# pgvector/pgvector

Measured on AMD Instinct MI355X. Metric: QPS @ recall@10 (IVFFlat, 1M x 1536d), higher is better.
Workload: dtype f32

## Files before the change

### pgvector_amd/csrc/kernels_query.hip

```cpp
#include "pgv_device.h"
#include "pgv_select.h"

#include <type_traits>

namespace pgv {

namespace {

constexpr int kQThreads = kSelThreads;
constexpr int kQWaves = kQThreads / kWave;
constexpr int kMaxBatchLists = 256;
constexpr int kHeadCap = 1024;

template <typename T, int METRIC, int NCH> struct WholeRows {
    Raw16 q[NCH];
    __device__ __forceinline__ void load_query(const char *qp, int lane) {
#pragma unroll
        for (int c = 0; c < NCH; c++) q[c] = load16(qp + ((size_t)c * kWave + lane) * sizeof(Raw16));
    }
    __device__ __forceinline__ float pair(const char *a, const char *b, int lane) const {
        Raw16 ra[NCH], rb[NCH];
#pragma unroll
        for (int c = 0; c < NCH; c++) ra[c] = load16(a + ((size_t)c * kWave + lane) * sizeof(Raw16));
#pragma unroll
// ... 290 lines not shown
        } else {
            out_dist[o] = INFINITY;
            if (out_slot) out_slot[o] = -1;
            if (out_tid) out_tid[o] = ~0ull;
        }
    }
    if (stats && threadIdx.x == 0) {
        atomicAdd(&stats[0], (double)m);
        atomicAdd(&stats[1], (double)m);
        atomicAdd(&stats[5], (double)m);
    }
}

constexpr int kRecheckCap = 256;

template <typename T, bool DOT = false>
__global__ __launch_bounds__(kQThreads) void batch_recheck_kernel(
    const char *__restrict__ vectors, const uint64_t *__restrict__ tids, int nvec, int lg,
    const char *__restrict__ queries, int kprime, int k, const float *__restrict__ approx_val,
    const int64_t *__restrict__ cand_pos, const int64_t *__restrict__ cand_slot,
    const int64_t *__restrict__ list_off, const int32_t *__restrict__ probe_lists,
    const int64_t *__restrict__ probe_off, int probes,
    const int64_t *__restrict__ seg_start, int64_t fixed_len,
    const unsigned *__restrict__ row_norm_max, ScanBound bound, const float *__restrict__ eps_add, int nq,
    float *__restrict__ out_dist, int64_t *__restrict__ out_slot, uint64_t *__restrict__ out_tid,
    int32_t *__restrict__ out_i32, int32_t *__restrict__ flags, float *__restrict__ pair_t, PlanEmit emit) {
    static_assert(!DOT || std::is_same<T, float>::value, "pair terms: fp32 rows");
    __shared__ float exact[kRecheckCap];
    __shared__ float dots[DOT ? kRecheckCap : 1];
    __shared__ __attribute__((aligned(16))) unsigned long long ent[kRecheckCap];
    const int q = blockIdx.x;
    const size_t row_bytes = (size_t)nvec * sizeof(Raw16);
    const int64_t m = seg_start ? seg_start[q + 1] - seg_start[q] : fixed_len;
    const int ncand = (int)(m < kprime ? m : (int64_t)kprime);
    const int kk = ncand < k ? ncand : k;
    const float *av = approx_val + (size_t)q * kprime;
    __shared__ float qn_part[kQWaves];
    {
        const char *qrow = queries + (size_t)q * row_bytes;
        float a = 0.f;
        for (int v = threadIdx.x; v < nvec; v += kQThreads) {
            const Raw16 x = load16(qrow + (size_t)v * sizeof(Raw16));
            a = accum_slice<T, 1>(a, x, x);
        }
        for (int m2 = 32; m2 > 0; m2 >>= 1) a += __shfl_xor(a, m2);
        if ((threadIdx.x & (kWave - 1)) == 0) qn_part[threadIdx.x >> 6] = a;
    }
    __syncthreads();
    float qn = 0.f;
    for (int w = 0; w < kQWaves; w++) qn += qn_part[w];
    const float rn = __uint_as_float(*row_norm_max);
    const float cross = 2.f * sqrtf(qn * rn);
    const float eps = 1.001f * (bound.g_sq * (qn + rn + cross) + bound.g_dot * cross + bound.g_norm * rn +
                                (eps_add ? eps_add[q] : 0.f));
    unsigned band = 0u;
    if (kk > 0) {
        const float edge = av[kk - 1] + 2.f * eps;
        band = float_to_key(edge + bound.g_ref * fabsf(edge + qn));
    }
    const int cnt = __syncthreads_count((int)threadIdx.x < ncand && float_to_key(av[threadIdx.x]) <= band);
    __shared__ int64_t slots[kRecheckCap];
    if ((int)threadIdx.x < cnt) {
        const int64_t p = cand_pos[(size_t)q * kprime + threadIdx.x];
        int64_t slot = p;
        if (cand_slot) {
            slot = cand_slot[(size_t)q * kprime + threadIdx.x];
        } else {
            const int64_t *off = probe_off + (size_t)q * probes;
            int lo = 0, hi = probes - 1;
            while (lo < hi) {
                const int mid = (lo + hi + 1) >> 1;
                if (off[mid] <= p)
                    lo = mid;
                else
                    hi = mid - 1;
            }
            slot = list_off[probe_lists[(size_t)q * probes + lo]] + (p - off[lo]);
        }
        slots[threadIdx.x] = slot;
    }
    __syncthreads();
    if constexpr (DOT)
        score_rows_dot([&](int64_t j) { return vectors + (size_t)slots[j] * row_bytes; }, 0, cnt,
                       queries + (size_t)q * row_bytes, nvec, lg, exact, dots);
    else
        score_rows<T, 0, 0>([&](int64_t j) { return vectors + (size_t)slots[j] * row_bytes; }, 0, cnt,
                            queries + (size_t)q * row_bytes, nvec, lg, exact);
    __syncthreads();
    if ((int)threadIdx.x < kRecheckCap)
        ent[threadIdx.x] = (int)threadIdx.x < cnt
                               ? ((unsigned long long)float_to_key(exact[threadIdx.x]) << 32) |
                                     (unsigned)cand_pos[(size_t)q * kprime + threadIdx.x]
                               : ~0ull;
    __syncthreads();
    const unsigned long long mine = ent[threadIdx.x];
    const int64_t my_slot = (int)threadIdx.x < cnt ? slots[threadIdx.x] : -1;
    int rank = 0;
    {
        const ulonglong2 *e2 = reinterpret_cast<const ulonglong2 *>(ent);
        const int n2 = (cnt + 1) / 2;
#pragma unroll 8
        for (int j = 0; j < n2; j++) {
            const ulonglong2 o = e2[j];
            rank += o.x < mine ? 1 : 0;
            rank += o.y < mine ? 1 : 0;
        }
    }
// ... 392 lines not shown
    float *cand_val = nullptr;
    int64_t *cand_pos = nullptr;
    int32_t *flags = nullptr;
    int carve(DBuf &buf, int nq, int kprime) {
        const size_t nk = (size_t)nq * kprime;
        const size_t a1 = (sizeof(float) * nk + 15) & ~(size_t)15, a2 = a1 + sizeof(int64_t) * nk;
        PGV_TRY(buf.ensure(a2 + sizeof(int32_t) * (2 * (size_t)nq + 1)));
        cand_val = buf.as<float>();
        cand_pos = reinterpret_cast<int64_t *>(buf.as<char>() + a1);
        flags = reinterpret_cast<int32_t *>(buf.as<char>() + a2);
        return PGV_OK;
    }
};
}

int launch_exact_tail(pgv_ctx *ctx, const ExactTail &t, DBuf &scratch) {
    if (t.nq <= 0) return PGV_OK;
    const ExactRows &xr = t.rows;
    const bool dense = t.dense();
    if (dense ? (t.fixed_len <= 0 || t.probe_off || t.seg_start || t.probes != 0)
              : (t.fixed_len != 0 || !t.probe_off || !t.seg_start || t.probes < 1))
        PGV_FAIL(PGV_ERR_ARG, "exact tail: a list plan or one dense run");
    if (t.kprime > kRecheckCap || t.k > t.kprime)
        PGV_FAIL(PGV_ERR_ARG, "exact tail: k' = %d outside k..%d", t.kprime, kRecheckCap);
    if (t.pair_t && xr.dtype != PGV_F32) PGV_FAIL(PGV_ERR_ARG, "exact tail: pair terms are for fp32 rows");
    static_assert(kWide >= kRecheckCap, "k <= k' <= kWide: batch_fix_kernel's emit");
    if (t.emit.cnt && !(dense && t.pair_t && t.out_i32 && t.emit.probe_off && t.emit.seg_len && t.emit.list_off))
        PGV_FAIL(PGV_ERR_ARG, "exact tail: the plan is counted where the pair terms are written");
    ApproxScratch sc;
    PGV_TRY(sc.carve(scratch, t.nq, t.kprime));
    const int64_t *cand_slot = dense ? sc.cand_pos : nullptr;
    const int64_t *seg_start = dense ? nullptr : t.seg_start;
    const int64_t fixed_len = dense ? t.fixed_len : 0;
    PGV_TRY(launch_topk_segments(ctx, t.approx, seg_start, t.nq, fixed_len, t.kprime, sc.cand_val, sc.cand_pos,
                                 sc.flags + t.nq, t.emit.cnt, t.emit.cnt ? 2 * (int)fixed_len : 0));
#define PGV_RECHECK(T, DOT)                                                                                          \
    hipLaunchKernelGGL((batch_recheck_kernel<T, DOT>), dim3(t.nq), dim3(kQThreads), 0, ctx->stream,                   \
                       static_cast<const char *>(xr.vectors), xr.tids, xr.geom.nvec, xr.geom.lpr_log2,                \
                       static_cast<const char *>(t.queries), t.kprime, t.k, sc.cand_val, sc.cand_pos, cand_slot,      \
                       xr.list_offsets, t.probe_lists, t.probe_off, t.probes, seg_start, fixed_len, xr.norm_max,      \
                       t.bound, t.eps_add, t.nq, t.out_dist, t.out_slot, t.out_tid, t.out_i32, sc.flags, t.pair_t,    \
                       t.emit)
    if (t.pair_t)
        PGV_RECHECK(float, true);
    else if (xr.dtype == PGV_F32)
        PGV_RECHECK(float, false);
    else
        PGV_RECHECK(__half, false);
#undef PGV_RECHECK
    PGV_HIP(hipGetLastError());
    double *stats = (ctx->profiling && ctx->stats_dev.p) ? ctx->stats_dev.as<double>() : nullptr;
    int kp = 2;
    while (kp < t.k) kp <<= 1;
    const int cap = kp > kFastCap ? kp : kFastCap;
    const size_t lds = (size_t)cap * 8 + sizeof(SelShared);
    const int grid = t.nq < ctx->num_cus ? t.nq : ctx->num_cus;
#define PGV_FIX(T)                                                                                                    \
    hipLaunchKernelGGL(batch_fix_kernel<T>, dim3(grid), dim3(kQThreads), lds, ctx->stream,                            \
                       static_cast<const char *>(xr.vectors), xr.list_offsets, xr.tids, xr.geom.nvec,                 \
                       xr.geom.lpr_log2, static_cast<const char *>(t.queries), t.probe_lists, t.probe_off, t.probes,  \
                       seg_start, fixed_len, sc.flags, t.nq, t.approx, t.k, kp, cap, xr.norm_max, t.bound, t.eps_add, \
                       ctx->no_widen ? 0 : 1, t.out_dist, t.out_slot, t.out_tid, t.out_i32, stats, t.pair_t, t.emit)
    if (xr.dtype == PGV_F32)
// ... 10 lines not shown
```

### pgvector_amd/csrc/kernels_select.hip

```cpp
#include "pgv_device.h"
#include "pgv_select.h"

namespace pgv {

namespace {


__global__ void plan_count_kernel(const int32_t *__restrict__ probe_lists,
                                  const int64_t *__restrict__ list_off, int nq, int probes,
                                  int *__restrict__ cnt, int64_t *__restrict__ probe_off,
                                  int64_t *__restrict__ seg_len) {
    const int q = blockIdx.x * blockDim.x + threadIdx.x;
    if (q >= nq) return;
    int64_t run = 0;
    for (int p = 0; p < probes; p++) {
        const int l = probe_lists[(size_t)q * probes + p];
        probe_off[(size_t)q * probes + p] = run;
        run += list_off[l + 1] - list_off[l];
        atomicAdd(&cnt[l], 1);
    }
    seg_len[q] = run;
}

template <typename F>
// ... 127 lines not shown
        ScanTask task;
        task.row0 = list_off[l] + (int64_t)c * rows_per_task;
        const int64_t left = len - (int64_t)c * rows_per_task;
        task.nrows = (int)(left < rows_per_task ? left : rows_per_task);
        task.pair0 = (int)(pair_start[l] + (int64_t)g * qt);
        const int pl = cnt[l] - g * qt;
        task.npairs = pl < qt ? pl : qt;
        task.pad = ng > 1 ? 1 : 0;
        tasks[t] = task;
    }
}

__global__ void plan_tasks_kernel(const int *__restrict__ cnt, const int64_t *__restrict__ list_off,
                                  const int64_t *__restrict__ pair_start,
                                  const int64_t *__restrict__ task_start, int nlists, int qt,
                                  int rows_per_task, ScanTask *__restrict__ tasks) {
    plan_tasks_body((int64_t)blockIdx.x * blockDim.x + threadIdx.x, (int64_t)gridDim.x * blockDim.x, cnt, list_off,
                    pair_start, task_start, nlists, qt, rows_per_task, tasks);
}

__global__ void plan_pairs_tasks_kernel(const int32_t *__restrict__ probe_lists, const int64_t *__restrict__ list_off,
                                        const int64_t *__restrict__ probe_off, const int64_t *__restrict__ seg_start,
                                        const int64_t *__restrict__ pair_start, const int64_t *__restrict__ task_start,
                                        const int *__restrict__ cnt, int *__restrict__ fill, int nq, int probes, int nlists,
                                        int qt, int rows_per_task, const float *__restrict__ pair_t, int pair_blocks,
                                        ScanPair *__restrict__ pairs, ScanTask *__restrict__ tasks) {
    if ((int)blockIdx.x < pair_blocks)
        plan_pairs_body((int64_t)blockIdx.x * blockDim.x + threadIdx.x, probe_lists, list_off, probe_off, seg_start,
                        pair_start, fill, nq, probes, pair_t, pairs);
    else
        plan_tasks_body((int64_t)(blockIdx.x - pair_blocks) * blockDim.x + threadIdx.x,
                        (int64_t)(gridDim.x - pair_blocks) * blockDim.x, cnt, list_off, pair_start, task_start, nlists, qt,
                        rows_per_task, tasks);
}

__device__ __forceinline__ bool dist_before(float a, float b) { return float_to_key(a) < float_to_key(b); }


__global__ __launch_bounds__(kSelThreads) void topk_kernel(
    const float *__restrict__ vals, const int64_t *__restrict__ seg_start, int64_t fixed_len,
    int k, int kp, int cap, float *__restrict__ out_val, int64_t *__restrict__ out_pos,
// ... 141 lines not shown
    const size_t nb = npairs + (size_t)nq + (size_t)nq + 1 + 2 * ((size_t)nlists + 1) + 3;
    PGV_TRY(ctx->plan_b.ensure(sizeof(int64_t) * nb));
    pb->cnt = ctx->plan_a.as<int>();
    pb->fill = pb->cnt + nlists;
    pb->probe_off = ctx->plan_b.as<int64_t>();
    pb->seg_len = pb->probe_off + npairs;
    pb->seg_start = pb->seg_len + nq;
    pb->pair_start = pb->seg_start + nq + 1;
    pb->task_start = pb->pair_start + nlists + 1;
    pb->totals = pb->task_start + nlists + 1;
    return PGV_OK;
}

int launch_plan_batch(pgv_ctx *ctx, const pgv_index *ix, const int32_t *probe_lists, int nq,
                      int probes, int qt, int rows_per_task, bool read_totals, PlanResult *res, const float *pair_t,
                      bool counted) {
    const int nlists = ix->nlists;
    const size_t npairs = (size_t)nq * probes;

    int64_t max_chunks = 0, sum_chunks = 0;
    for (int l = 0; l < nlists; l++) {
        const int64_t nc = (ix->h_offsets[l + 1] - ix->h_offsets[l] + rows_per_task - 1) / rows_per_task;
        sum_chunks += nc;
        if (nc > max_chunks) max_chunks = nc;
    }
    res->ntasks_bound = max_chunks * (int64_t)(npairs / qt) + sum_chunks;
    res->out_bound = (int64_t)nq * ix->len_prefix[probes];
    if (res->ntasks_bound > 0x7fffffff) PGV_FAIL(PGV_ERR_ARG, "plan: too many tasks");

    PlanBuffers pb;
    PGV_TRY(plan_batch_reserve(ctx, nlists, nq, probes, &pb));
// ... 8 lines not shown
    const unsigned task_blocks = (unsigned)(want < 1 ? 1 : (want > cap ? cap : want));
    const unsigned pair_blocks = (unsigned)((npairs + 255) / 256);
    res->ntasks = res->ntasks_bound;
    res->total_out = res->out_bound;

    if (counted) {
        double *acc = nullptr;
        if (read_totals) {
            PGV_TRY(ctx->stats_dev.ensure(8 * sizeof(double)));
            acc = ctx->stats_dev.as<double>();
        }
        hipLaunchKernelGGL(plan_scan_kernel, dim3(1), dim3(1024), 0, ctx->stream, cnt, ix->list_offsets, seg_len, nq, nlists,
                           qt, rows_per_task, seg_start, pair_start, task_start, totals, acc);
        hipLaunchKernelGGL(plan_pairs_tasks_kernel, dim3(pair_blocks + task_blocks), dim3(256), 0, ctx->stream, probe_lists,
                           ix->list_offsets, probe_off, seg_start, pair_start, task_start, cnt, fill, nq, probes, nlists, qt,
                           rows_per_task, pair_t, (int)pair_blocks, ctx->pairs.as<ScanPair>(), tasks);
        PGV_HIP(hipGetLastError());
    } else {
        PGV_HIP(hipMemsetAsync(cnt, 0, sizeof(int) * 2 * (size_t)nlists, ctx->stream));
        hipLaunchKernelGGL(plan_count_kernel, dim3((nq + 255) / 256), dim3(256), 0, ctx->stream,
                           probe_lists, ix->list_offsets, nq, probes, cnt, probe_off, seg_len);
        hipLaunchKernelGGL(plan_scan_kernel, dim3(1), dim3(1024), 0, ctx->stream, cnt,
                           ix->list_offsets, seg_len, nq, nlists, qt, rows_per_task, seg_start,
                           pair_start, task_start, totals, static_cast<double *>(nullptr));
        hipLaunchKernelGGL(plan_pairs_kernel, dim3(pair_blocks), dim3(256), 0,
                           ctx->stream, probe_lists, ix->list_offsets, probe_off, seg_start,
                           pair_start, fill, nq, probes, pair_t, ctx->pairs.as<ScanPair>());
        hipLaunchKernelGGL(plan_tasks_kernel, dim3(task_blocks), dim3(256), 0,
                           ctx->stream, cnt, ix->list_offsets, pair_start, task_start, nlists, qt, rows_per_task, tasks);
        PGV_HIP(hipGetLastError());
        if (read_totals) {
            PGV_TRY(ctx->stats_dev.ensure(8 * sizeof(double)));
            hipLaunchKernelGGL(plan_stats_kernel, dim3(1), dim3(256), 0, ctx->stream, cnt,
                               ix->list_offsets, totals, nlists, qt, ctx->stats_dev.as<double>());
            PGV_HIP(hipGetLastError());
        }
    }
    res->tasks = tasks;
    res->pairs = ctx->pairs.as<ScanPair>();
    res->ntasks_dev = reinterpret_cast<int *>(totals + 2);
    res->seg_start = seg_start;
    res->probe_off = probe_off;
    res->pair_start = pair_start;
    return PGV_OK;
// ... 41 lines not shown
```

### pgvector_amd/csrc/kernels_shadow.hip

```cpp
#include "pgv_device.h"

#include <cfloat>

namespace pgv {

namespace {

__device__ __forceinline__ int list_of_row(const int64_t *__restrict__ list_off, int nlists, int64_t r) {
    int lo = 0, hi = nlists - 1;
    while (lo < hi) {
        const int mid = (lo + hi + 1) >> 1;
        if (list_off[mid] <= r)
            lo = mid;
        else
            hi = mid - 1;
    }
    return lo;
}

__device__ __forceinline__ int scale_for(float m) {
    if (!(m > 0.f) || !isfinite(m)) return 0;
    int e;
    (void)frexpf(m, &e);
    return e - 14;
// ... 105 lines not shown
            qq[e & 3] = fma(xi, xi, qq[e & 3]);
            dd[e & 3] = fma(xi - back, xi - back, dd[e & 3]);
            hh[e & 3] = fma(back, back, hh[e & 3]);
        }
        out.v[e] = v;
    }
    *reinterpret_cast<uint4 *>(h + 8 * c) = out.w;
}

__global__ __launch_bounds__(256) void shadow_query_kernel(const float *__restrict__ queries, int nq, int ld, int ld16,
                                                           ShadowTerms st, RankShadowTerms rt,
                                                           const float *__restrict__ center_norm_max,
                                                           const float *__restrict__ row_norm_max,
                                                           __half *__restrict__ qcast, float *__restrict__ qscale,
                                                           float *__restrict__ qeps, float *__restrict__ cscale,
                                                           float *__restrict__ ceps) {
    const int q = (int)(blockIdx.x * 4 + (threadIdx.x >> 6));
    if (q >= nq) return;
    const int lane = threadIdx.x & (kWave - 1);
    const float *x = queries + (size_t)q * ld;
    __half *h = qcast + (size_t)q * ld16;
    const int nchunks = ld16 / 8;
    const bool in_regs = nchunks <= kWave * kCastChunks;
    CastChunk reg[kCastChunks];
    float m = 0.f;
    if (in_regs) {
#pragma unroll
        for (int j = 0; j < kCastChunks; j++) {
            const int c = lane + j * kWave;
            reg[j] = cast_chunk_load(x, c < nchunks ? c : nchunks, ld);
        }
// ... 92 lines not shown
    hipLaunchKernelGGL(shadow_build_kernel, grid, dim3(256), 0, ctx->stream, static_cast<const float *>(rows),
                       static_cast<const float *>(centers), list_off, nlists, n, g32.ld, g16.ld, max_bits, static_cast<__half *>(shadow), ep);
    PGV_HIP(hipGetLastError());
    return PGV_OK;
}

int shadow_scale_of(float max_abs) {
    if (!(max_abs > 0.f) || !std::isfinite(max_abs)) return 0;
    int e;
    (void)std::frexp(max_abs, &e);
    return e - 14;
}

int launch_shadow_query(pgv_ctx *ctx, const RowGeom &g32, const RowGeom &g16, const void *queries, int nq,
                        const ShadowTerms &st, const RankShadowTerms &rt, const float *center_norm_max,
                        const float *row_norm_max, void *qcast, float *qscale, float *qeps, float *cscale, float *ceps) {
    if (nq <= 0) return PGV_OK;
    hipLaunchKernelGGL(shadow_query_kernel, dim3((unsigned)((nq + 3) / 4)), dim3(256), 0, ctx->stream,
                       static_cast<const float *>(queries), nq, g32.ld, g16.ld, st, rt, center_norm_max, row_norm_max,
                       static_cast<__half *>(qcast), qscale, qeps, cscale, ceps);
    PGV_HIP(hipGetLastError());
    return PGV_OK;
}

int launch_shadow_pairs(pgv_ctx *ctx, const RowGeom &g32, const void *queries, const void *centers,
                        const int64_t *pair_start, int nlists, int64_t npairs, ScanPair *pairs) {
    if (npairs <= 0) return PGV_OK;
    hipLaunchKernelGGL(shadow_pair_kernel, dim3((unsigned)((npairs + 3) / 4)), dim3(256), 0, ctx->stream,
                       static_cast<const float *>(queries), static_cast<const float *>(centers), pair_start, nlists, npairs,
                       g32.ld, pairs);
    PGV_HIP(hipGetLastError());
    return PGV_OK;
}

}
// ... 1 lines not shown
```

### pgvector_amd/csrc/pgv_abi_ivf.hip

```cpp
#include "pgv_abi_common.h"

extern "C" {


namespace {
struct IndexLayout {
    size_t centers, vectors, offsets, tids, row_norms, center_norms, bytes;
    bool has_tids, has_norms;
};
IndexLayout index_layout(int nlists, int64_t n, size_t row_bytes, bool has_tids, bool l2) {
    auto up = [](size_t v) { return (v + 255) & ~(size_t)255; };
    IndexLayout L{};
    size_t at = 0;
    L.centers = at; at = up(at + (size_t)nlists * row_bytes);
    L.vectors = at; at = up(at + (size_t)(n > 0 ? n : 1) * row_bytes);
    L.offsets = at; at = up(at + sizeof(int64_t) * ((size_t)nlists + 1));
    L.has_tids = has_tids;
    L.tids = at; if (has_tids) at = up(at + sizeof(uint64_t) * (size_t)n);
    L.has_norms = l2;
    L.row_norms = at; if (l2 && n > 0) at = up(at + sizeof(float) * ((size_t)n + 1));
    L.center_norms = at; if (l2) at = up(at + sizeof(float) * ((size_t)nlists + 1));
    L.bytes = at;
    return L;
}
// ... 92 lines not shown
        ix->cshadow_P = Pc * (1.0 + 1e-9);
    }
    return PGV_OK;
}

struct ShadowBatch {
    void *qcast = nullptr;
    float *qscale = nullptr, *qeps = nullptr;
    float *cscale = nullptr, *ceps = nullptr;
    float *pair_t = nullptr;
    bool scan_follows = false;
    bool cast_for_scan = false;
    bool pairs_done = false;
};

int shadow_batch_cast(pgv_index *ix, const void *q_dev, int nq, int probes, bool for_rank, bool for_scan, ShadowBatch *sb) {
    pgv_ctx *ctx = ix->ctx;
    const RowGeom &g16 = ix->shadow_geom;
    const size_t qb = ((size_t)nq * g16.ld * sizeof(uint16_t) + 255) & ~(size_t)255;
    PGV_TRY(ctx->sh_q.ensure(qb + sizeof(float) * (size_t)nq * (4 + (size_t)probes)));
    sb->qcast = ctx->sh_q.p;
    sb->qscale = reinterpret_cast<float *>(ctx->sh_q.as<char>() + qb);
    sb->qeps = sb->qscale + nq;
    sb->cscale = sb->qeps + nq;
    sb->ceps = sb->cscale + nq;
    sb->pair_t = sb->ceps + nq;
    constexpr double u = 5.9604644775390625e-8;
    ShadowTerms st{};
    st.s = ix->shadow_s;
    st.E = ix->shadow_E;
    st.P = ix->shadow_P;
    st.g_dot = gamma_n(shadow_chain_length(g16) + 4.0, u);
    st.g_pair = gamma_n((double)pair_chain_length(ix->geom), u);
    st.g_cn = shadow_band(ix->geom.ld, 0.f, u).g_norm;
    RankShadowTerms rt{};
    rt.s = ix->cshadow_s;
    rt.E = ix->cshadow_E;
    rt.P = ix->cshadow_P;
    rt.g_dot = st.g_dot;
    rt.g_cn = st.g_cn;
    PGV_TRY(launch_shadow_query(ctx, ix->geom, g16, q_dev, nq, st, rt, ix->center_norms + ix->nlists,
                                ix->row_norms + ix->nrows, sb->qcast, for_scan ? sb->qscale : nullptr,
                                for_scan ? sb->qeps : nullptr, for_rank ? sb->cscale : nullptr,
                                for_rank ? sb->ceps : nullptr));
    sb->cast_for_scan = for_scan;
    return PGV_OK;
}

template <typename Fill>
int index_create(pgv_ctx *ctx, pgv_metric metric, pgv_dtype dtype, int dim, int nlists, const std::vector<int64_t> &off,
                 bool has_tids, Fill fill, pgv_index **out) {
    const int64_t n = off[nlists];
    pgv_index *ix = new (std::nothrow) pgv_index();
    if (!ix) PGV_FAIL(PGV_ERR_NOMEM, "out of host memory");
    ix->ctx = ctx;
    ix->refs = new (std::nothrow) int(1);
    if (!ix->refs) {
        delete ix;
        PGV_FAIL(PGV_ERR_NOMEM, "out of host memory");
// ... 599 lines not shown
        const int64_t cd_stride = ((int64_t)ix->nlists + 7) / 4 * 4;
        PGV_TRY(ctx->dist_mat.ensure(sizeof(float) * (size_t)nq * cd_stride));
        return launch_multi_rank(ctx, ix, q_dev, nq, ctx->dist_mat.as<float>(), cd_stride, maxprobes, out_lists_dev,
                                 out_dist_dev);
    }
    int cand = maxprobes + 16 < ix->nlists ? maxprobes + 16 : ix->nlists;
    const int rank_env = rank_shadow_env();
    const bool rank_sh = ix->metric == PGV_L2SQ && ix->cshadow && ix->dtype == PGV_F32 && rank_env != 0 && shadow_env() != 0;
    if (rank_sh && maxprobes + 54 <= 256) cand = maxprobes + 54 < ix->nlists ? maxprobes + 54 : ix->nlists;
    const bool mfma = nq >= 128 && ix->nlists >= 64 && !ctx->no_mfma_scan &&
                      (ix->metric == PGV_NEG_IP || (ix->metric == PGV_L2SQ && ix->center_norms && cand <= 256));
    if (mfma && ix->metric == PGV_L2SQ) {
        ShadowBatch own;
        if (!sb) sb = &own;
        const bool scan_follows = sb->scan_follows;
        if (rank_sh) {
            PGV_TRY(shadow_batch_cast(ix, q_dev, nq, maxprobes, true, scan_follows, sb));
            PGV_TRY(dense_scan(ctx, ix->metric, PGV_F16, ix->shadow_geom, ix->cshadow, ix->nlists, sb->qcast, nq, ix->nlists,
                               mat, true, ix->center_norms, nullptr, sb->cscale));
        } else {
            PGV_TRY(dense_scan(ctx, ix->metric, ix->dtype, ix->geom, ix->centers, ix->nlists, q_dev, nq, ix->nlists, mat,
                               true, ix->center_norms, nullptr));
        }
        ExactTail tail;
        tail.pair_t = (rank_sh && rank_env == 1 && scan_follows) ? sb->pair_t : nullptr;
        PlanBuffers pbuf;
        if (tail.pair_t) {
            PGV_TRY(plan_batch_reserve(ctx, ix->nlists, nq, maxprobes, &pbuf));
            tail.emit = {pbuf.cnt, pbuf.probe_off, pbuf.seg_len, ix->list_offsets};
        }
        tail.rows = {ix->centers, nullptr, nullptr, ix->geom, ix->dtype,
                     reinterpret_cast<const unsigned *>(ix->center_norms + ix->nlists)};
        tail.queries = q_dev;
        tail.nq = nq;
        tail.kprime = cand;
        tail.k = maxprobes;
        tail.approx = mat;
        tail.fixed_len = ix->nlists;
        tail.bound = scan_bound_chain(ctx, ix->geom.ld, scan_chain_length(ix->geom, ix->dtype, false));
        if (rank_sh) tail.bound = shadow_band(ix->geom.ld, tail.bound.g_ref);
        tail.eps_add = rank_sh ? sb->ceps : nullptr;
        tail.out_dist = dist;
        tail.out_i32 = out_lists_dev;
        PGV_TRY(launch_exact_tail(ctx, tail, ctx->ms_b));
// ... 184 lines not shown
        PGV_TRY(launch_multi_scan(ctx, ix, q_dev, nq, probe_lists, probes, bound, ctx->plan_d.as<float>(), seg_stride, k,
                                  od.as<float>(), os.as<int64_t>(), ot.as<uint64_t>()));
        PGV_TRY(timer.end());
        PGV_TRY(scan_turn_end(ctx));
        bool need = false;
        PGV_TRY(od.finish(ctx, &need));
        PGV_TRY(os.finish(ctx, &need));
        PGV_TRY(ot.finish(ctx, &need));
        return sync_if(ctx, need);
    }
    ShadowBatch own;
    if (!sb) sb = &own;
    if (path.shadow && !sb->cast_for_scan) PGV_TRY(shadow_batch_cast(ix, q_dev, nq, probes, false, true, sb));
    const float *pair_t = (path.shadow && sb->pairs_done) ? sb->pair_t : nullptr;
    PlanResult plan;
    PGV_TRY(launch_plan_batch(ctx, ix, probe_lists, nq, probes, path.qt, path.rows_per_task, ctx->profiling, &plan, pair_t,
                              pair_t != nullptr));
    if (path.shadow) {
        if (!pair_t)
            PGV_TRY(launch_shadow_pairs(ctx, ix->geom, q_dev, ix->centers, plan.pair_start, ix->nlists, (int64_t)nq * probes,
                                        plan.pairs));
        ctx->scan_shadow_queries += nq;
    }

    PGV_TRY(ctx->plan_d.ensure(sizeof(float) * (size_t)(plan.out_bound > 0 ? plan.out_bound : 1)));
    float *seg_vals = ctx->plan_d.as<float>();
    if (plan.ntasks_bound > 0) {
        PGV_TRY(scan_turn_begin(ctx));
        ScanTimer timer{ctx};
        PGV_TRY(timer.begin(0.0, 0.0));
        if (path.shadow)
            PGV_TRY(launch_mfma_scan(ctx, ix->metric, PGV_F16, ix->shadow_geom, ix->shadow, sb->qcast, plan.tasks,
// ... 26 lines not shown
        tail.queries = q_dev;
        tail.nq = nq;
        tail.kprime = approx_candidates(k);
        tail.k = k;
        tail.approx = seg_vals;
        tail.probe_lists = probe_lists;
        tail.probe_off = plan.probe_off;
        tail.probes = probes;
        tail.seg_start = plan.seg_start;
        tail.bound = scan_bound_chain(ctx, ix->geom.ld, scan_chain_length(ix->geom, ix->dtype, path.wide));
        if (path.shadow) tail.bound = shadow_band(ix->geom.ld, tail.bound.g_ref);
        tail.eps_add = path.shadow ? sb->qeps : nullptr;
        tail.out_dist = od.as<float>();
        tail.out_slot = os.as<int64_t>();
        tail.out_tid = ot.as<uint64_t>();
        PGV_TRY(launch_exact_tail(ctx, tail, ctx->ms_a));
    } else {
        PGV_TRY(launch_topk_segments(ctx, seg_vals, plan.seg_start, nq, 0, k, od.as<float>(), pos));
        PGV_TRY(launch_positions_to_slots(ctx, ix, probe_lists, plan.probe_off, nq, probes, k, pos,
                                          os.as<int64_t>(), ot.as<uint64_t>()));
    }
    bool need = false;
    PGV_TRY(od.finish(ctx, &need));
    PGV_TRY(os.finish(ctx, &need));
    PGV_TRY(ot.finish(ctx, &need));
    return sync_if(ctx, need);
}

int scan_batch_dev(pgv_index *ix, const void *q_dev, int nq, const int32_t *probe_lists, int probes, int k, float *out_dist,
                   int64_t *out_slot, uint64_t *out_tid) {
// ... 284 lines not shown
```

### pgvector_amd/csrc/pgv_internal.h

```cpp
#pragma once

#include <hip/hip_runtime.h>

#include <cstdint>
#include <cstdio>
#include <cstdlib>
#include <cstring>
#include <cmath>
#include <vector>

#include "../../include/pgv_hip.h"

namespace pgv {

void set_error(const char *fmt, ...) __attribute__((format(printf, 1, 2)));

#define PGV_FAIL(code, ...)            \
    do {                               \
        ::pgv::set_error(__VA_ARGS__); \
        return (code);                 \
    } while (0)

#define PGV_HIP(call)                                                                  \
    do {                                                                               \
// ... 352 lines not shown
int mfma_scan_queries_per_task();
int launch_mfma_dense(pgv_ctx *ctx, pgv_metric metric, pgv_dtype dtype, const RowGeom &g, const void *rows, int64_t n,
                      const void *queries, int nq, const float *row_norms, float *out, int64_t out_stride);
int dense_chain_length(const RowGeom &g, pgv_dtype dtype);
int launch_row_norms(pgv_ctx *ctx, pgv_dtype dtype, const RowGeom &g, const void *rows, int64_t n, float *out,
                     unsigned *max_bits);
int launch_mfma_scan(pgv_ctx *ctx, pgv_metric metric, pgv_dtype dtype, const RowGeom &g, const void *rows,
                     const void *queries, const ScanTask *tasks, const int *ntasks_dev, int ntasks_bound,
                     const ScanPair *pairs, const float *row_norms, const float *query_norms, float *out, bool stream_rows,
                     int queries_per_task = 32, const float *shadow_scale = nullptr);
int launch_shadow_build(pgv_ctx *ctx, const RowGeom &g32, const RowGeom &g16, const void *rows, const void *centers,
                        const int64_t *list_off, int nlists, int64_t n, void *shadow, void *words);
int shadow_scale_of(float max_abs);
int shadow_chain_length(const RowGeom &g16);
int scan_chain_length(const RowGeom &g, pgv_dtype dtype, bool wide);
int launch_shadow_query(pgv_ctx *ctx, const RowGeom &g32, const RowGeom &g16, const void *queries, int nq,
                        const ShadowTerms &st, const RankShadowTerms &rt, const float *center_norm_max,
                        const float *row_norm_max, void *qcast, float *qscale, float *qeps, float *cscale, float *ceps);
int launch_shadow_pairs(pgv_ctx *ctx, const RowGeom &g32, const void *queries, const void *centers,
                        const int64_t *pair_start, int nlists, int64_t npairs, ScanPair *pairs);
int mfma_scan_queries_per_task_wide();

int launch_gather_words(pgv_ctx *ctx, const void *src, int words_per_row, int64_t nrows, const int64_t *idx, int n,
                        uint32_t *out);
size_t build_sort_scratch_bytes(int64_t n, int key_bits);
int launch_build_order(pgv_ctx *ctx, const int32_t *lists, int64_t n, int nlists, unsigned long long *keys_tmp,
                       unsigned long long *keys_sorted, unsigned long long *counts, int64_t *offsets, int *bad,
                       void *sort_scratch, size_t sort_scratch_bytes);
int launch_build_gather(pgv_ctx *ctx, const void *src_rows, const unsigned long long *keys_sorted, int64_t n, int nvec,
                        void *dst_rows, const uint64_t *src_tids, uint64_t *dst_tids);

struct PlanResult {
    ScanTask *tasks = nullptr;
// ... 8 lines not shown
    int64_t *pair_start = nullptr;
};
struct PlanBuffers {
    int *cnt = nullptr, *fill = nullptr;
    int64_t *probe_off = nullptr, *seg_len = nullptr;
    int64_t *seg_start = nullptr, *pair_start = nullptr, *task_start = nullptr, *totals = nullptr;
};
int plan_batch_reserve(pgv_ctx *ctx, int nlists, int nq, int probes, PlanBuffers *pb);
struct PlanEmit {
    int *cnt = nullptr;
    int64_t *probe_off = nullptr, *seg_len = nullptr;
    const int64_t *list_off = nullptr;
};
int launch_plan_batch(pgv_ctx *ctx, const pgv_index *ix, const int32_t *probe_lists, int nq,
                      int probes, int qt, int rows_per_task, bool read_totals, PlanResult *res,
                      const float *pair_t = nullptr, bool counted = false);
int launch_topk_segments(pgv_ctx *ctx, const float *vals, const int64_t *seg_start, int nseg,
                         int64_t fixed_len, int k, float *out_val, int64_t *out_pos, int32_t *zero_word = nullptr,
                         int32_t *zero_range = nullptr, int zero_n = 0);
int launch_positions_to_slots(pgv_ctx *ctx, const pgv_index *ix, const int32_t *probe_lists,
                              const int64_t *probe_off, int nq, int probes, int k,
                              const int64_t *pos, int64_t *out_slot, uint64_t *out_tid);
struct ExactRows {
    const void *vectors;
    const uint64_t *tids;
    const int64_t *list_offsets;
    pgv::RowGeom geom;
    pgv_dtype dtype;
    const unsigned *norm_max;
};
struct ExactTail {
// ... 4 lines not shown
    int k = 0;
    float *approx = nullptr;
    const int32_t *probe_lists = nullptr;
    const int64_t *probe_off = nullptr;
    int probes = 0;
    const int64_t *seg_start = nullptr;
    int64_t fixed_len = 0;
    ScanBound bound{};
    const float *eps_add = nullptr;
    float *out_dist = nullptr;
    int64_t *out_slot = nullptr;
    uint64_t *out_tid = nullptr;
    int32_t *out_i32 = nullptr;
    float *pair_t = nullptr;
    PlanEmit emit;
    bool dense() const { return probe_lists == nullptr; }
};
int launch_exact_tail(pgv_ctx *ctx, const ExactTail &t, DBuf &scratch);
int launch_iota_slots(pgv_ctx *ctx, const pgv_index *ix, const int32_t *lists_dev, int nlists,
                      const int64_t *probe_off, int64_t *out_slot);

int query_max_batch_lists();
int query_head_cap();
size_t query_head_bytes(int head);
int launch_query_stage(pgv_ctx *ctx, const void *src_pinned, void *dst_dev, int nvec);
int launch_multi_rank(pgv_ctx *ctx, const pgv_index *ix, const void *q_dev, int nq, float *cdist, int64_t cd_stride,
                      int max_probes, int32_t *out_lists, float *out_dist);
int launch_multi_scan(pgv_ctx *ctx, const pgv_index *ix, const void *q_dev, int nq, const int32_t *probe_lists, int nprobes,
                      int64_t rows_bound, float *seg, int64_t seg_stride, int k, float *out_dist, int64_t *out_slot,
                      uint64_t *out_tid);
int launch_query_iota(pgv_ctx *ctx, int32_t *out, int n);
int launch_one_query_rows(pgv_ctx *ctx, pgv_metric metric, pgv_dtype dtype, const RowGeom &g, const void *rows, int n,
// ... 44 lines not shown
```

Baseline: 1.373 million.

## Fuse segment top-k selection into the exact recheck kernel

Folds the per-query segment top-k selection into the batch recheck kernel, so candidates come straight from shared memory instead of a separate launch writing cand_val/cand_pos to global scratch. The zeroing of the flag and count words moves into earlier kernels (shadow query cast, plan tasks). Probe offsets and list bases are staged in LDS for the binary search, and query-norm loads are hoisted ahead of the selection. This removes a kernel launch and a global round trip per batch, at the cost of more dynamic shared memory per workgroup and a more complex kernel with possibly lower occupancy.

```diff
diff --git a/pgvector_amd/csrc/kernels_query.hip b/pgvector_amd/csrc/kernels_query.hip
--- a/pgvector_amd/csrc/kernels_query.hip
+++ b/pgvector_amd/csrc/kernels_query.hip
@@ -328,7 +328,10 @@
 
 constexpr int kRecheckCap = 256;
 
-template <typename T, bool DOT = false>
+constexpr int kProbeLds = 128;
+constexpr int kQnHoist = 2;
+
+template <typename T, bool DOT = false, bool FUSED = false>
 __global__ __launch_bounds__(kQThreads) void batch_recheck_kernel(
     const char *__restrict__ vectors, const uint64_t *__restrict__ tids, int nvec, int lg,
     const char *__restrict__ queries, int kprime, int k, const float *__restrict__ approx_val,
@@ -338,22 +341,67 @@
     const int64_t *__restrict__ seg_start, int64_t fixed_len,
     const unsigned *__restrict__ row_norm_max, ScanBound bound, const float *__restrict__ eps_add, int nq,
     float *__restrict__ out_dist, int64_t *__restrict__ out_slot, uint64_t *__restrict__ out_tid,
-    int32_t *__restrict__ out_i32, int32_t *__restrict__ flags, float *__restrict__ pair_t, PlanEmit emit) {
+    int32_t *__restrict__ out_i32, int32_t *__restrict__ flags, float *__restrict__ pair_t, PlanEmit emit, int kp, int cap) {
     static_assert(!DOT || std::is_same<T, float>::value, "pair terms: fp32 rows");
+    static_assert(kQThreads == kSelThreads && kRecheckCap <= kQThreads, "one workgroup selects and rechecks a query");
+    extern __shared__ __attribute__((aligned(16))) char smem[];
     __shared__ float exact[kRecheckCap];
     __shared__ float dots[DOT ? kRecheckCap : 1];
     __shared__ __attribute__((aligned(16))) unsigned long long ent[kRecheckCap];
+    __shared__ int64_t poff[FUSED ? kProbeLds : 1], pbase[FUSED ? kProbeLds : 1];
     const int q = blockIdx.x;
     const size_t row_bytes = (size_t)nvec * sizeof(Raw16);
-    const int64_t m = seg_start ? seg_start[q + 1] - seg_start[q] : fixed_len;
+    const int64_t seg_base = seg_start ? seg_start[q] : (int64_t)q * fixed_len;
+    const int64_t m = seg_start ? seg_start[q + 1] - seg_base : fixed_len;
     const int ncand = (int)(m < kprime ? m : (int64_t)kprime);
     const int kk = ncand < k ? ncand : k;
     const float *av = approx_val + (size_t)q * kprime;
+    const bool dense = FUSED ? probe_lists == nullptr : cand_slot != nullptr;
+    const bool lds_probes = FUSED && !dense && probes <= kProbeLds;
+    float av_mine = INFINITY, av_edge = INFINITY;
+    int64_t pos_mine = -1;
     __shared__ float qn_part[kQWaves];
     {
         const char *qrow = queries + (size_t)q * row_bytes;
         float a = 0.f;
-        for (int v = threadIdx.x; v < nvec; v += kQThreads) {
+        int v = threadIdx.x;
+        if constexpr (FUSED) {
+            Raw16 x[kQnHoist];
+#pragma unroll
+            for (int h = 0; h < kQnHoist; h++) {
+                const int at = v + h * kQThreads;
+                x[h] = load16(qrow + (size_t)(at < nvec ? at : 0) * sizeof(Raw16));
+            }
+            int64_t off_r = 0;
+            int32_t list_r = 0;
+            if (lds_probes && (int)threadIdx.x < probes) {
+                off_r = probe_off[(size_t)q * probes + threadIdx.x];
+                list_r = probe_lists[(size_t)q * probes + threadIdx.x];
+            }
+            unsigned long long *sel_ent = reinterpret_cast<unsigned long long *>(smem);
+            SelShared *sel = reinterpret_cast<SelShared *>(smem + (size_t)cap * 8);
+            block_topk_auto(approx_val + seg_base, m, kprime, kp, cap, sel_ent, sel);
+            __syncthreads();
+            if (lds_probes && (int)threadIdx.x < probes) {
+                poff[threadIdx.x] = off_r;
+                pbase[threadIdx.x] = list_off[list_r];
+            }
+            auto value_of = [&](int i) {
+                const unsigned long long e = sel_ent[i];
+                return (e != ~0ull && i < ncand) ? key_to_float((unsigned)(e >> 32)) : INFINITY;
+            };
+            if ((int)threadIdx.x < kprime) {
+                const unsigned long long e = sel_ent[threadIdx.x];
+                av_mine = value_of((int)threadIdx.x);
+                pos_mine = (e != ~0ull && (int)threadIdx.x < ncand) ? (int64_t)(unsigned)(e & 0xffffffffu) : -1;
+            }
+            if (kk > 0) av_edge = value_of(kk - 1);
+#pragma unroll
+            for (int h = 0; h < kQnHoist; h++)
+                if (v + h * kQThreads < nvec) a = accum_slice<T, 1>(a, x[h], x[h]);
+            v += kQnHoist * kQThreads;
+        }
+        for (; v < nvec; v += kQThreads) {
             const Raw16 x = load16(qrow + (size_t)v * sizeof(Raw16));
             a = accum_slice<T, 1>(a, x, x);
         }
@@ -369,16 +417,29 @@
                                 (eps_add ? eps_add[q] : 0.f));
     unsigned band = 0u;
     if (kk > 0) {
-        const float edge = av[kk - 1] + 2.f * eps;
+        const float edge = (FUSED ? av_edge : av[kk - 1]) + 2.f * eps;
         band = float_to_key(edge + bound.g_ref * fabsf(edge + qn));
     }
-    const int cnt = __syncthreads_count((int)threadIdx.x < ncand && float_to_key(av[threadIdx.x]) <= band);
+    if constexpr (!FUSED)
+        if ((int)threadIdx.x < ncand) av_mine = av[threadIdx.x];
+    const int cnt = __syncthreads_count((int)threadIdx.x < ncand && float_to_key(av_mine) <= band);
     __shared__ int64_t slots[kRecheckCap];
     if ((int)threadIdx.x < cnt) {
-        const int64_t p = cand_pos[(size_t)q * kprime + threadIdx.x];
+        if constexpr (!FUSED) pos_mine = cand_pos[(size_t)q * kprime + threadIdx.x];
+        const int64_t p = pos_mine;
         int64_t slot = p;
-        if (cand_slot) {
-            slot = cand_slot[(size_t)q * kprime + threadIdx.x];
+        if (dense) {
+            if constexpr (!FUSED) slot = cand_slot[(size_t)q * kprime + threadIdx.x];
+        } else if (lds_probes) {
+            int lo = 0, hi = probes - 1;
+            while (lo < hi) {
+                const int mid = (lo + hi + 1) >> 1;
+                if (poff[mid] <= p)
+                    lo = mid;
+                else
+                    hi = mid - 1;
+            }
+            slot = pbase[lo] + (p - poff[lo]);
         } else {
             const int64_t *off = probe_off + (size_t)q * probes;
             int lo = 0, hi = probes - 1;
@@ -403,8 +464,7 @@
     __syncthreads();
     if ((int)threadIdx.x < kRecheckCap)
         ent[threadIdx.x] = (int)threadIdx.x < cnt
-                               ? ((unsigned long long)float_to_key(exact[threadIdx.x]) << 32) |
-                                     (unsigned)cand_pos[(size_t)q * kprime + threadIdx.x]
+                               ? ((unsigned long long)float_to_key(exact[threadIdx.x]) << 32) | (unsigned)pos_mine
                                : ~0ull;
     __syncthreads();
     const unsigned long long mine = ent[threadIdx.x];
@@ -827,6 +887,21 @@
 };
 }
 
+bool exact_tail_fused() {
+    static const bool on = [] {
+        const char *e = getenv("PGV_TAIL_FUSED");
+        return e ? atoi(e) != 0 : true;
+    }();
+    return on;
+}
+
+int exact_tail_reserve(DBuf &scratch, int nq, int32_t **count) {
+    ApproxScratch sc;
+    PGV_TRY(sc.carve(scratch, nq, 0));
+    *count = sc.flags + nq;
+    return PGV_OK;
+}
+
 int launch_exact_tail(pgv_ctx *ctx, const ExactTail &t, DBuf &scratch) {
     if (t.nq <= 0) return PGV_OK;
     const ExactRows &xr = t.rows;
@@ -840,26 +915,41 @@
     static_assert(kWide >= kRecheckCap, "k <= k' <= kWide: batch_fix_kernel's emit");
     if (t.emit.cnt && !(dense && t.pair_t && t.out_i32 && t.emit.probe_off && t.emit.seg_len && t.emit.list_off))
         PGV_FAIL(PGV_ERR_ARG, "exact tail: the plan is counted where the pair terms are written");
+    const bool fused = exact_tail_fused() && t.cleared_count != nullptr;
     ApproxScratch sc;
-    PGV_TRY(sc.carve(scratch, t.nq, t.kprime));
-    const int64_t *cand_slot = dense ? sc.cand_pos : nullptr;
+    PGV_TRY(sc.carve(scratch, t.nq, fused ? 0 : t.kprime));
+    if (fused && t.cleared_count != sc.flags + t.nq)
+        PGV_FAIL(PGV_ERR_STATE, "exact tail: the scratch moved after its flagged-query count was cleared");
     const int64_t *seg_start = dense ? nullptr : t.seg_start;
     const int64_t fixed_len = dense ? t.fixed_len : 0;
-    PGV_TRY(launch_topk_segments(ctx, t.approx, seg_start, t.nq, fixed_len, t.kprime, sc.cand_val, sc.cand_pos,
-                                 sc.flags + t.nq, t.emit.cnt, t.emit.cnt ? 2 * (int)fixed_len : 0));
-#define PGV_RECHECK(T, DOT)                                                                                          \
-    hipLaunchKernelGGL((batch_recheck_kernel<T, DOT>), dim3(t.nq), dim3(kQThreads), 0, ctx->stream,                   \
+    int skp = 2;
+    while (skp < t.kprime) skp <<= 1;
+    const int scap = skp > kFastCap ? skp : kFastCap;
+    const size_t slds = fused ? (size_t)scap * 8 + sizeof(SelShared) : 0;
+    const int64_t *cand_slot = (dense && !fused) ? sc.cand_pos : nullptr;
+    if (!fused)
+        PGV_TRY(launch_topk_segments(ctx, t.approx, seg_start, t.nq, fixed_len, t.kprime, sc.cand_val, sc.cand_pos,
+                                     sc.flags + t.nq, t.emit.cnt, t.emit.cnt ? 2 * (int)fixed_len : 0));
+#define PGV_RECHECK(T, DOT, FUSED)                                                                                   \
+    hipLaunchKernelGGL((batch_recheck_kernel<T, DOT, FUSED>), dim3(t.nq), dim3(kQThreads), slds, ctx->stream,         \
                        static_cast<const char *>(xr.vectors), xr.tids, xr.geom.nvec, xr.geom.lpr_log2,                \
-                       static_cast<const char *>(t.queries), t.kprime, t.k, sc.cand_val, sc.cand_pos, cand_slot,      \
-                       xr.list_offsets, t.probe_lists, t.probe_off, t.probes, seg_start, fixed_len, xr.norm_max,      \
-                       t.bound, t.eps_add, t.nq, t.out_dist, t.out_slot, t.out_tid, t.out_i32, sc.flags, t.pair_t,    \
-                       t.emit)
-    if (t.pair_t)
-        PGV_RECHECK(float, true);
-    else if (xr.dtype == PGV_F32)
-        PGV_RECHECK(float, false);
-    else
-        PGV_RECHECK(__half, false);
+                       static_cast<const char *>(t.queries), t.kprime, t.k, FUSED ? t.approx : sc.cand_val,           \
+                       sc.cand_pos, cand_slot, xr.list_offsets, t.probe_lists, t.probe_off, t.probes, seg_start,      \
+                       fixed_len, xr.norm_max, t.bound, t.eps_add, t.nq, t.out_dist, t.out_slot, t.out_tid,           \
+                       t.out_i32, sc.flags, t.pair_t, t.emit, skp, scap)
+#define PGV_RECHECK_T(FUSED)              \
+    if (t.pair_t)                         \
+        PGV_RECHECK(float, true, FUSED);  \
+    else if (xr.dtype == PGV_F32)         \
+        PGV_RECHECK(float, false, FUSED); \
+    else                                  \
+        PGV_RECHECK(__half, false, FUSED)
+    if (fused) {
+        PGV_RECHECK_T(true);
+    } else {
+        PGV_RECHECK_T(false);
+    }
+#undef PGV_RECHECK_T
 #undef PGV_RECHECK
     PGV_HIP(hipGetLastError());
     double *stats = (ctx->profiling && ctx->stats_dev.p) ? ctx->stats_dev.as<double>() : nullptr;
diff --git a/pgvector_amd/csrc/kernels_select.hip b/pgvector_amd/csrc/kernels_select.hip
--- a/pgvector_amd/csrc/kernels_select.hip
+++ b/pgvector_amd/csrc/kernels_select.hip
@@ -165,7 +165,8 @@
 __global__ void plan_tasks_kernel(const int *__restrict__ cnt, const int64_t *__restrict__ list_off,
                                   const int64_t *__restrict__ pair_start,
                                   const int64_t *__restrict__ task_start, int nlists, int qt,
-                                  int rows_per_task, ScanTask *__restrict__ tasks) {
+                                  int rows_per_task, ScanTask *__restrict__ tasks, int32_t *__restrict__ zero_word) {
+    if (zero_word && blockIdx.x == 0 && threadIdx.x == 0) *zero_word = 0;
     plan_tasks_body((int64_t)blockIdx.x * blockDim.x + threadIdx.x, (int64_t)gridDim.x * blockDim.x, cnt, list_off,
                     pair_start, task_start, nlists, qt, rows_per_task, tasks);
 }
@@ -175,7 +176,9 @@
                                         const int64_t *__restrict__ pair_start, const int64_t *__restrict__ task_start,
                                         const int *__restrict__ cnt, int *__restrict__ fill, int nq, int probes, int nlists,
                                         int qt, int rows_per_task, const float *__restrict__ pair_t, int pair_blocks,
-                                        ScanPair *__restrict__ pairs, ScanTask *__restrict__ tasks) {
+                                        ScanPair *__restrict__ pairs, ScanTask *__restrict__ tasks,
+                                        int32_t *__restrict__ zero_word) {
+    if (zero_word && blockIdx.x == 0 && threadIdx.x == 0) *zero_word = 0;
     if ((int)blockIdx.x < pair_blocks)
         plan_pairs_body((int64_t)blockIdx.x * blockDim.x + threadIdx.x, probe_lists, list_off, probe_off, seg_start,
                         pair_start, fill, nq, probes, pair_t, pairs);
@@ -347,7 +350,7 @@
 
 int launch_plan_batch(pgv_ctx *ctx, const pgv_index *ix, const int32_t *probe_lists, int nq,
                       int probes, int qt, int rows_per_task, bool read_totals, PlanResult *res, const float *pair_t,
-                      bool counted) {
+                      bool counted, int32_t *zero_word) {
     const int nlists = ix->nlists;
     const size_t npairs = (size_t)nq * probes;
 
@@ -386,7 +389,7 @@
                            qt, rows_per_task, seg_start, pair_start, task_start, totals, acc);
         hipLaunchKernelGGL(plan_pairs_tasks_kernel, dim3(pair_blocks + task_blocks), dim3(256), 0, ctx->stream, probe_lists,
                            ix->list_offsets, probe_off, seg_start, pair_start, task_start, cnt, fill, nq, probes, nlists, qt,
-                           rows_per_task, pair_t, (int)pair_blocks, ctx->pairs.as<ScanPair>(), tasks);
+                           rows_per_task, pair_t, (int)pair_blocks, ctx->pairs.as<ScanPair>(), tasks, zero_word);
         PGV_HIP(hipGetLastError());
     } else {
         PGV_HIP(hipMemsetAsync(cnt, 0, sizeof(int) * 2 * (size_t)nlists, ctx->stream));
@@ -399,7 +402,8 @@
                            ctx->stream, probe_lists, ix->list_offsets, probe_off, seg_start,
                            pair_start, fill, nq, probes, pair_t, ctx->pairs.as<ScanPair>());
         hipLaunchKernelGGL(plan_tasks_kernel, dim3(task_blocks), dim3(256), 0,
-                           ctx->stream, cnt, ix->list_offsets, pair_start, task_start, nlists, qt, rows_per_task, tasks);
+                           ctx->stream, cnt, ix->list_offsets, pair_start, task_start, nlists, qt, rows_per_task, tasks,
+                           zero_word);
         PGV_HIP(hipGetLastError());
         if (read_totals) {
             PGV_TRY(ctx->stats_dev.ensure(8 * sizeof(double)));
diff --git a/pgvector_amd/csrc/kernels_shadow.hip b/pgvector_amd/csrc/kernels_shadow.hip
--- a/pgvector_amd/csrc/kernels_shadow.hip
+++ b/pgvector_amd/csrc/kernels_shadow.hip
@@ -143,7 +143,10 @@
                                                            const float *__restrict__ row_norm_max,
                                                            __half *__restrict__ qcast, float *__restrict__ qscale,
                                                            float *__restrict__ qeps, float *__restrict__ cscale,
-                                                           float *__restrict__ ceps) {
+                                                           float *__restrict__ ceps, StreamClear clear) {
+    if (clear.word && blockIdx.x == 0 && threadIdx.x == 0) *clear.word = 0;
+    if (clear.range)
+        for (int i = (int)(blockIdx.x * 256 + threadIdx.x); i < clear.n; i += (int)(gridDim.x * 256)) clear.range[i] = 0;
     const int q = (int)(blockIdx.x * 4 + (threadIdx.x >> 6));
     if (q >= nq) return;
     const int lane = threadIdx.x & (kWave - 1);
@@ -266,11 +269,12 @@
 
 int launch_shadow_query(pgv_ctx *ctx, const RowGeom &g32, const RowGeom &g16, const void *queries, int nq,
                         const ShadowTerms &st, const RankShadowTerms &rt, const float *center_norm_max,
-                        const float *row_norm_max, void *qcast, float *qscale, float *qeps, float *cscale, float *ceps) {
+                        const float *row_norm_max, void *qcast, float *qscale, float *qeps, float *cscale, float *ceps,
+                        StreamClear clear) {
     if (nq <= 0) return PGV_OK;
     hipLaunchKernelGGL(shadow_query_kernel, dim3((unsigned)((nq + 3) / 4)), dim3(256), 0, ctx->stream,
                        static_cast<const float *>(queries), nq, g32.ld, g16.ld, st, rt, center_norm_max, row_norm_max,
-                       static_cast<__half *>(qcast), qscale, qeps, cscale, ceps);
+                       static_cast<__half *>(qcast), qscale, qeps, cscale, ceps, clear);
     PGV_HIP(hipGetLastError());
     return PGV_OK;
 }
diff --git a/pgvector_amd/csrc/pgv_abi_ivf.hip b/pgvector_amd/csrc/pgv_abi_ivf.hip
--- a/pgvector_amd/csrc/pgv_abi_ivf.hip
+++ b/pgvector_amd/csrc/pgv_abi_ivf.hip
@@ -130,7 +130,8 @@
     bool pairs_done = false;
 };
 
-int shadow_batch_cast(pgv_index *ix, const void *q_dev, int nq, int probes, bool for_rank, bool for_scan, ShadowBatch *sb) {
+int shadow_batch_cast(pgv_index *ix, const void *q_dev, int nq, int probes, bool for_rank, bool for_scan, ShadowBatch *sb,
+                      StreamClear clear = {}) {
     pgv_ctx *ctx = ix->ctx;
     const RowGeom &g16 = ix->shadow_geom;
     const size_t qb = ((size_t)nq * g16.ld * sizeof(uint16_t) + 255) & ~(size_t)255;
@@ -158,7 +159,7 @@
     PGV_TRY(launch_shadow_query(ctx, ix->geom, g16, q_dev, nq, st, rt, ix->center_norms + ix->nlists,
                                 ix->row_norms + ix->nrows, sb->qcast, for_scan ? sb->qscale : nullptr,
                                 for_scan ? sb->qeps : nullptr, for_rank ? sb->cscale : nullptr,
-                                for_rank ? sb->ceps : nullptr));
+                                for_rank ? sb->ceps : nullptr, clear));
     sb->cast_for_scan = for_scan;
     return PGV_OK;
 }
@@ -788,20 +789,28 @@
         ShadowBatch own;
         if (!sb) sb = &own;
         const bool scan_follows = sb->scan_follows;
+        ExactTail tail;
+        const bool want_pairs = rank_sh && rank_env == 1 && scan_follows;
+        PlanBuffers pbuf;
+        if (want_pairs) {
+            PGV_TRY(plan_batch_reserve(ctx, ix->nlists, nq, maxprobes, &pbuf));
+            tail.emit = {pbuf.cnt, pbuf.probe_off, pbuf.seg_len, ix->list_offsets};
+        }
         if (rank_sh) {
-            PGV_TRY(shadow_batch_cast(ix, q_dev, nq, maxprobes, true, scan_follows, sb));
+            StreamClear clear;
+            if (exact_tail_fused()) {
+                PGV_TRY(exact_tail_reserve(ctx->ms_b, nq, &clear.word));
+                clear.range = tail.emit.cnt;
+                clear.n = tail.emit.cnt ? 2 * ix->nlists : 0;
+                tail.cleared_count = clear.word;
+            }
+            PGV_TRY(shadow_batch_cast(ix, q_dev, nq, maxprobes, true, scan_follows, sb, clear));
+            if (want_pairs) tail.pair_t = sb->pair_t;
             PGV_TRY(dense_scan(ctx, ix->metric, PGV_F16, ix->shadow_geom, ix->cshadow, ix->nlists, sb->qcast, nq, ix->nlists,
                                mat, true, ix->center_norms, nullptr, sb->cscale));
         } else {
             PGV_TRY(dense_scan(ctx, ix->metric, ix->dtype, ix->geom, ix->centers, ix->nlists, q_dev, nq, ix->nlists, mat,
                                true, ix->center_norms, nullptr));
-        }
-        ExactTail tail;
-        tail.pair_t = (rank_sh && rank_env == 1 && scan_follows) ? sb->pair_t : nullptr;
-        PlanBuffers pbuf;
-        if (tail.pair_t) {
-            PGV_TRY(plan_batch_reserve(ctx, ix->nlists, nq, maxprobes, &pbuf));
-            tail.emit = {pbuf.cnt, pbuf.probe_off, pbuf.seg_len, ix->list_offsets};
         }
         tail.rows = {ix->centers, nullptr, nullptr, ix->geom, ix->dtype,
                      reinterpret_cast<const unsigned *>(ix->center_norms + ix->nlists)};
@@ -1016,8 +1025,10 @@
     if (path.shadow && !sb->cast_for_scan) PGV_TRY(shadow_batch_cast(ix, q_dev, nq, probes, false, true, sb));
     const float *pair_t = (path.shadow && sb->pairs_done) ? sb->pair_t : nullptr;
     PlanResult plan;
+    int32_t *tail_count = nullptr;
+    if (path.approx && exact_tail_fused()) PGV_TRY(exact_tail_reserve(ctx->ms_a, nq, &tail_count));
     PGV_TRY(launch_plan_batch(ctx, ix, probe_lists, nq, probes, path.qt, path.rows_per_task, ctx->profiling, &plan, pair_t,
-                              pair_t != nullptr));
+                              pair_t != nullptr, tail_count));
     if (path.shadow) {
         if (!pair_t)
             PGV_TRY(launch_shadow_pairs(ctx, ix->geom, q_dev, ix->centers, plan.pair_start, ix->nlists, (int64_t)nq * probes,
@@ -1074,6 +1085,7 @@
         tail.out_dist = od.as<float>();
         tail.out_slot = os.as<int64_t>();
         tail.out_tid = ot.as<uint64_t>();
+        tail.cleared_count = tail_count;
         PGV_TRY(launch_exact_tail(ctx, tail, ctx->ms_a));
     } else {
         PGV_TRY(launch_topk_segments(ctx, seg_vals, plan.seg_start, nq, 0, k, od.as<float>(), pos));
diff --git a/pgvector_amd/csrc/pgv_internal.h b/pgvector_amd/csrc/pgv_internal.h
--- a/pgvector_amd/csrc/pgv_internal.h
+++ b/pgvector_amd/csrc/pgv_internal.h
@@ -390,9 +390,15 @@
 int shadow_scale_of(float max_abs);
 int shadow_chain_length(const RowGeom &g16);
 int scan_chain_length(const RowGeom &g, pgv_dtype dtype, bool wide);
+struct StreamClear {
+    int32_t *word = nullptr;
+    int32_t *range = nullptr;
+    int n = 0;
+};
 int launch_shadow_query(pgv_ctx *ctx, const RowGeom &g32, const RowGeom &g16, const void *queries, int nq,
                         const ShadowTerms &st, const RankShadowTerms &rt, const float *center_norm_max,
-                        const float *row_norm_max, void *qcast, float *qscale, float *qeps, float *cscale, float *ceps);
+                        const float *row_norm_max, void *qcast, float *qscale, float *qeps, float *cscale, float *ceps,
+                        StreamClear clear = {});
 int launch_shadow_pairs(pgv_ctx *ctx, const RowGeom &g32, const void *queries, const void *centers,
                         const int64_t *pair_start, int nlists, int64_t npairs, ScanPair *pairs);
 int mfma_scan_queries_per_task_wide();
@@ -431,7 +437,7 @@
 };
 int launch_plan_batch(pgv_ctx *ctx, const pgv_index *ix, const int32_t *probe_lists, int nq,
                       int probes, int qt, int rows_per_task, bool read_totals, PlanResult *res,
-                      const float *pair_t = nullptr, bool counted = false);
+                      const float *pair_t = nullptr, bool counted = false, int32_t *zero_word = nullptr);
 int launch_topk_segments(pgv_ctx *ctx, const float *vals, const int64_t *seg_start, int nseg,
                          int64_t fixed_len, int k, float *out_val, int64_t *out_pos, int32_t *zero_word = nullptr,
                          int32_t *zero_range = nullptr, int zero_n = 0);
@@ -466,8 +472,11 @@
     int32_t *out_i32 = nullptr;
     float *pair_t = nullptr;
     PlanEmit emit;
+    const int32_t *cleared_count = nullptr;
     bool dense() const { return probe_lists == nullptr; }
 };
+bool exact_tail_fused();
+int exact_tail_reserve(DBuf &scratch, int nq, int32_t **count);
 int launch_exact_tail(pgv_ctx *ctx, const ExactTail &t, DBuf &scratch);
 int launch_iota_slots(pgv_ctx *ctx, const pgv_index *ix, const int32_t *lists_dev, int nlists,
                       const int64_t *probe_off, int64_t *out_slot);
```

Result: no change. 1.369 million (-0.3%).
